# ai-dynamo/dynamo

Measured on AMD Instinct MI355X. Metric: output tok/s (node), Llama-3-70B serving, ISL8192/OSL1024, conc 16/GPU, higher is better.
Workload: dtype bf16; 1 GPU; model=llama-3-70b, global_batch=16, seq_len=8192, osl=1024, parallelism=agg1, kv_cache_dtype=auto

## Files before the change

### dynamo_amd/csrc/bindings.cpp

```cpp
#include <torch/extension.h>
#include <pybind11/pybind11.h>

namespace py = pybind11;

void rmsnorm(torch::Tensor out, torch::Tensor input, torch::Tensor weight, double eps);
void fused_add_rmsnorm(torch::Tensor input, torch::Tensor residual,
                       torch::Tensor weight, double eps);
void rope_append_qkv(torch::Tensor q_out, torch::Tensor kcache,
                     torch::Tensor vcache, torch::Tensor qkv,
                     c10::optional<torch::Tensor> bias,
                     torch::Tensor positions, torch::Tensor slot_mapping,
                     torch::Tensor cos_sin_cache, bool v_transposed);
void rope_inplace(torch::Tensor q, torch::Tensor k, torch::Tensor positions,
                  torch::Tensor cos_sin_cache, int64_t num_q_heads,
                  int64_t num_k_heads, int64_t head_dim);
void silu_mul(torch::Tensor out, torch::Tensor gate_up);
void gelu(torch::Tensor out, torch::Tensor input);
void kv_cache_append(torch::Tensor kcache, torch::Tensor vcache, torch::Tensor k,
                     torch::Tensor v, torch::Tensor slot_mapping,
                     bool v_transposed);
void gather_pages(torch::Tensor staging, torch::Tensor cache, torch::Tensor page_ids);
void scatter_pages(torch::Tensor staging, torch::Tensor cache, torch::Tensor page_ids);
void copy_pages(torch::Tensor dst_cache, torch::Tensor src_cache, torch::Tensor pairs);
int64_t paged_decode_num_chunks(int64_t max_ctx);
int64_t decode_chunk_tokens_py(int64_t max_ctx);
void paged_attention_decode(torch::Tensor out, torch::Tensor q, torch::Tensor kcache,
                            torch::Tensor vcache, torch::Tensor page_table,
                            torch::Tensor ctx_lens, torch::Tensor partial,
                            torch::Tensor ml, double scale,
                            int64_t chunk_tokens, bool v_transposed,
                            c10::optional<torch::Tensor> chunk_cnt);
void attention_prefill_paged(torch::Tensor out, torch::Tensor q,
                             torch::Tensor kcache, torch::Tensor vcache,
                             torch::Tensor page_table, torch::Tensor tile_seq,
                             torch::Tensor tile_q0, torch::Tensor seq_q_start,
                             torch::Tensor seq_q_len, torch::Tensor seq_ctx_len,
                             double scale, bool v_transposed);
void greedy_sample(torch::Tensor out, torch::Tensor logits);
void topkp_sample(torch::Tensor out, torch::Tensor logits,
                  torch::Tensor inv_temp, torch::Tensor top_k,
                  torch::Tensor top_p, int64_t seed,
                  c10::optional<torch::Tensor> row_seeds);
void gumbel_sample(torch::Tensor out, torch::Tensor logits, torch::Tensor inv_temp,
                   int64_t seed, c10::optional<torch::Tensor> row_seeds);
void moe_grouped_gemm(torch::Tensor y, torch::Tensor x, torch::Tensor w,
                      torch::Tensor tiles);
void moe_grouped_gemm_seg(torch::Tensor y, torch::Tensor x, torch::Tensor w,
                          torch::Tensor seg_start, int64_t max_tokens);
void topk_gating(torch::Tensor topw, torch::Tensor topi, torch::Tensor logits);
torch::Tensor ipc_alloc(int64_t nbytes, int64_t device);
py::bytes ipc_export(torch::Tensor t);
torch::Tensor ipc_open(py::bytes handle_bytes, int64_t nbytes, int64_t device);
void enable_peer_access(int64_t device, int64_t peer);
torch::Tensor mfma_probe(torch::Tensor A, torch::Tensor B);
torch::Tensor tr16_probe();
torch::Tensor vstage_probe();
torch::Tensor pv_probe(int64_t hot);

PYBIND11_MODULE(TORCH_EXTENSION_NAME, m) {
  m.doc() = "dynamo_amd native MI355X (gfx950) kernels";
  m.def("rmsnorm", &rmsnorm);
  m.def("fused_add_rmsnorm", &fused_add_rmsnorm);
  m.def("rope_inplace", &rope_inplace);
  m.def("rope_append_qkv", &rope_append_qkv,
        py::arg("q_out"), py::arg("kcache"), py::arg("vcache"),
        py::arg("qkv"), py::arg("bias"), py::arg("positions"),
        py::arg("slot_mapping"), py::arg("cos_sin"),
        py::arg("v_transposed") = false);
  m.def("silu_mul", &silu_mul);
  m.def("gelu", &gelu);
  m.def("kv_cache_append", &kv_cache_append, py::arg("kcache"),
        py::arg("vcache"), py::arg("k"), py::arg("v"),
        py::arg("slot_mapping"), py::arg("v_transposed") = false);
  m.def("gather_pages", &gather_pages);
  m.def("scatter_pages", &scatter_pages);
  m.def("copy_pages", &copy_pages);
  m.def("paged_decode_num_chunks", &paged_decode_num_chunks);
  m.def("decode_chunk_tokens", &decode_chunk_tokens_py);
  m.def("paged_attention_decode", &paged_attention_decode,
        py::arg("out"), py::arg("q"), py::arg("kcache"), py::arg("vcache"),
        py::arg("page_table"), py::arg("ctx_lens"), py::arg("partial"),
        py::arg("ml"), py::arg("scale"), py::arg("chunk_tokens"),
        py::arg("v_transposed") = false,
        py::arg("chunk_cnt") = py::none());
  m.def("attention_prefill_paged", &attention_prefill_paged,
        py::arg("out"), py::arg("q"), py::arg("kcache"), py::arg("vcache"),
        py::arg("page_table"), py::arg("tile_seq"), py::arg("tile_q0"),
        py::arg("seq_q_start"), py::arg("seq_q_len"), py::arg("seq_ctx_len"),
        py::arg("scale"), py::arg("v_transposed") = false);
  m.def("greedy_sample", &greedy_sample);
  m.def("gumbel_sample", &gumbel_sample, py::arg("out"), py::arg("logits"),
        py::arg("inv_temp"), py::arg("seed"),
        py::arg("row_seeds") = py::none());
  m.def("topkp_sample", &topkp_sample, py::arg("out"), py::arg("logits"),
        py::arg("inv_temp"), py::arg("top_k"), py::arg("top_p"),
        py::arg("seed"), py::arg("row_seeds") = py::none());
  m.def("moe_grouped_gemm", &moe_grouped_gemm);
  m.def("moe_grouped_gemm_seg", &moe_grouped_gemm_seg);
  m.def("topk_gating", &topk_gating);
  m.def("ipc_alloc", &ipc_alloc);
  m.def("ipc_export", &ipc_export);
  m.def("ipc_open", &ipc_open);
  m.def("enable_peer_access", &enable_peer_access);
  m.def("mfma_probe", &mfma_probe);
  m.def("tr16_probe", &tr16_probe);
  m.def("vstage_probe", &vstage_probe);
  m.def("pv_probe", &pv_probe);
}
```

### dynamo_amd/csrc/norm.hip

```cpp
#include "common.h"
#include <torch/extension.h>
#include <ATen/hip/HIPContext.h>

namespace {

constexpr int kBlock = 256;

template <bool FUSED_ADD>
__global__ void rmsnorm_kernel(short* __restrict__ out,
                               short* __restrict__ x,
                               short* __restrict__ res,
                               const short* __restrict__ w,
                               float eps, int rows, int D) {
  __shared__ float lds[kBlock / WAVE_SIZE];
  const int nvec = D / 8;
  for (int row = blockIdx.x; row < rows; row += gridDim.x) {
    short* xrow = x + (int64_t)row * D;
    short* rrow = FUSED_ADD ? res + (int64_t)row * D : nullptr;
    short* orow = out + (int64_t)row * D;

    float ss = 0.f;
    for (int v = threadIdx.x; v < nvec; v += kBlock) {
      short8 xv = *reinterpret_cast<const short8*>(xrow + v * 8);
      if constexpr (FUSED_ADD) {
        short8 rv = *reinterpret_cast<const short8*>(rrow + v * 8);
        short8 sv;
#pragma unroll
        for (int i = 0; i < 8; i++) {
          float s = bf16_to_f32(xv[i]) + bf16_to_f32(rv[i]);
          sv[i] = f32_to_bf16(s);
          ss += s * s;
        }
        *reinterpret_cast<short8*>(rrow + v * 8) = sv;
      } else {
#pragma unroll
        for (int i = 0; i < 8; i++) {
          float xf = bf16_to_f32(xv[i]);
          ss += xf * xf;
        }
      }
    }
    ss = block_reduce_sum(ss, lds);
    const float inv = rsqrtf(ss / (float)D + eps);

    for (int v = threadIdx.x; v < nvec; v += kBlock) {
      const short* src = FUSED_ADD ? rrow : xrow;
      short8 sv = *reinterpret_cast<const short8*>(src + v * 8);
      short8 wv = *reinterpret_cast<const short8*>(w + v * 8);
      short8 ov;
#pragma unroll
      for (int i = 0; i < 8; i++)
        ov[i] = f32_to_bf16(bf16_to_f32(sv[i]) * inv * bf16_to_f32(wv[i]));
      *reinterpret_cast<short8*>(orow + v * 8) = ov;
    }
    __syncthreads();
  }
}

}

void rmsnorm(torch::Tensor out, torch::Tensor input, torch::Tensor weight, double eps) {
  TORCH_CHECK(input.is_cuda() && input.dtype() == torch::kBFloat16);
  TORCH_CHECK(input.is_contiguous() && out.is_contiguous());
  const int D = input.size(-1);
  const int rows = input.numel() / D;
  TORCH_CHECK(D % 8 == 0, "hidden size must be a multiple of 8");
  const int grid = std::min<int>(rows, 2048);
  if (rows == 0) return;
  auto stream = at::cuda::getCurrentHIPStream();
  rmsnorm_kernel<false><<<grid, kBlock, 0, stream>>>(
      (short*)out.data_ptr(), (short*)input.data_ptr(), nullptr,
      (const short*)weight.data_ptr(), (float)eps, rows, D);
  HIP_CHECK_KERNEL();
}

void fused_add_rmsnorm(torch::Tensor input, torch::Tensor residual,
                       torch::Tensor weight, double eps) {
  TORCH_CHECK(input.is_cuda() && input.dtype() == torch::kBFloat16);
  TORCH_CHECK(input.is_contiguous() && residual.is_contiguous());
  const int D = input.size(-1);
  const int rows = input.numel() / D;
  TORCH_CHECK(D % 8 == 0);
  const int grid = std::min<int>(rows, 2048);
  if (rows == 0) return;
  auto stream = at::cuda::getCurrentHIPStream();
  rmsnorm_kernel<true><<<grid, kBlock, 0, stream>>>(
      (short*)input.data_ptr(), (short*)input.data_ptr(),
      (short*)residual.data_ptr(), (const short*)weight.data_ptr(),
      (float)eps, rows, D);
  HIP_CHECK_KERNEL();
}
```

### dynamo_amd/csrc/rope.hip

```cpp
#include "common.h"
#include <hip/hip_fp8.h>
#include <torch/extension.h>
#include <ATen/hip/HIPContext.h>

namespace {

constexpr int kBlock = 256;

__global__ void rope_kernel(short* __restrict__ q,
                            short* __restrict__ k,
                            const int32_t* __restrict__ positions,
                            const float* __restrict__ cos_sin,
                            int T, int Hq, int Hk, int hd) {
  const int t = blockIdx.x;
  if (t >= T) return;
  const int half = hd / 2;
  const int pos = positions[t];
  const float* cs = cos_sin + (int64_t)pos * hd;

  const int total = (Hq + Hk) * (half / 8);
  for (int idx = threadIdx.x; idx < total; idx += kBlock) {
    const int h = idx / (half / 8);
    const int i0 = (idx % (half / 8)) * 8;
    short* base = (h < Hq) ? q + ((int64_t)t * Hq + h) * hd
                           : k + ((int64_t)t * Hk + (h - Hq)) * hd;
    short8 x1 = *reinterpret_cast<const short8*>(base + i0);
    short8 x2 = *reinterpret_cast<const short8*>(base + half + i0);
    float4v c0 = *reinterpret_cast<const float4v*>(cs + i0);
    float4v c1 = *reinterpret_cast<const float4v*>(cs + i0 + 4);
    float4v s0 = *reinterpret_cast<const float4v*>(cs + half + i0);
    float4v s1 = *reinterpret_cast<const float4v*>(cs + half + i0 + 4);
    short8 o1, o2;
#pragma unroll
    for (int i = 0; i < 8; i++) {
      float c = (i < 4) ? c0[i] : c1[i - 4];
      float s = (i < 4) ? s0[i] : s1[i - 4];
      float a = bf16_to_f32(x1[i]);
      float b = bf16_to_f32(x2[i]);
      o1[i] = f32_to_bf16(a * c - b * s);
      o2[i] = f32_to_bf16(b * c + a * s);
    }
    *reinterpret_cast<short8*>(base + i0) = o1;
    *reinterpret_cast<short8*>(base + half + i0) = o2;
  }
}

template <int FP8 = 0, int VT = 0>
__global__ void rope_append_kernel(
    short* __restrict__ q_out,
    short* __restrict__ kcache,
    short* __restrict__ vcache,
    const short* __restrict__ qkv,
    const short* __restrict__ bias,
    const int32_t* __restrict__ positions,
    const int64_t* __restrict__ slots,
    const float* __restrict__ cos_sin,
    int T, int Hq, int Hkv, int page_size, int hd, int row_stride) {
  const int t = blockIdx.x;
  if (t >= T) return;
  const int half = hd / 2;
  const int pos = positions[t];
  const float* cs = cos_sin + (int64_t)pos * hd;
  const short* row = qkv + (int64_t)t * row_stride;
  const int64_t slot = slots[t];
  const int64_t page = slot >= 0 ? slot / page_size : 0;
  const int off = slot >= 0 ? (int)(slot % page_size) : 0;

  const int rope_units = (Hq + Hkv) * (half / 8);
  for (int idx = threadIdx.x; idx < rope_units; idx += kBlock) {
    const int h = idx / (half / 8);
    const int i0 = (idx % (half / 8)) * 8;
    const int src_off = h * hd;
    short8 x1 = *reinterpret_cast<const short8*>(row + src_off + i0);
    short8 x2 = *reinterpret_cast<const short8*>(row + src_off + half + i0);
    float4v c0 = *reinterpret_cast<const float4v*>(cs + i0);
    float4v c1 = *reinterpret_cast<const float4v*>(cs + i0 + 4);
    float4v s0 = *reinterpret_cast<const float4v*>(cs + half + i0);
    float4v s1 = *reinterpret_cast<const float4v*>(cs + half + i0 + 4);
    short8 o1, o2;
#pragma unroll
    for (int i = 0; i < 8; i++) {
      const float c = (i < 4) ? c0[i] : c1[i - 4];
      const float s = (i < 4) ? s0[i] : s1[i - 4];
      float a = bf16_to_f32(x1[i]);
      float b = bf16_to_f32(x2[i]);
      if (bias) {
        a += bf16_to_f32(bias[src_off + i0 + i]);
        b += bf16_to_f32(bias[src_off + half + i0 + i]);
      }
      o1[i] = f32_to_bf16(a * c - b * s);
      o2[i] = f32_to_bf16(b * c + a * s);
    }
    if (h < Hq) {
      short* qb = q_out + ((int64_t)t * Hq + h) * hd;
      *reinterpret_cast<short8*>(qb + i0) = o1;
      *reinterpret_cast<short8*>(qb + half + i0) = o2;
    } else if (slot >= 0) {
      const int kh = h - Hq;
      const int64_t kb = ((page * Hkv + kh) * page_size + off) * hd;
      if constexpr (FP8) {
        unsigned char* kc8 = reinterpret_cast<unsigned char*>(kcache);
        uchar8 p1, p2;
#pragma unroll
        for (int e = 0; e < 8; e++) {
          p1[e] = __hip_cvt_float_to_fp8(bf16_to_f32(o1[e]),
                                         __HIP_SATFINITE, __HIP_E4M3);
          p2[e] = __hip_cvt_float_to_fp8(bf16_to_f32(o2[e]),
                                         __HIP_SATFINITE, __HIP_E4M3);
        }
        *reinterpret_cast<uchar8*>(kc8 + kb + i0) = p1;
        *reinterpret_cast<uchar8*>(kc8 + kb + half + i0) = p2;
      } else {
        *reinterpret_cast<short8*>(kcache + kb + i0) = o1;
        *reinterpret_cast<short8*>(kcache + kb + half + i0) = o2;
      }
    }
  }
  if (slot >= 0) {
    const int voff = (Hq + Hkv) * hd;
    const int nvec = Hkv * hd / 8;
    for (int i = threadIdx.x; i < nvec; i += kBlock) {
      const int h = (i * 8) / hd;
      const int d = (i * 8) % hd;
      short8 v = *reinterpret_cast<const short8*>(row + voff + h * hd + d);
      if (bias) {
#pragma unroll
        for (int e = 0; e < 8; e++)
          v[e] = f32_to_bf16(bf16_to_f32(v[e]) +
                             bf16_to_f32(bias[voff + h * hd + d + e]));
      }
      if constexpr (VT) {
        const int64_t vb0 = ((page * Hkv + h) * hd + d) * page_size + off;
#pragma unroll
        for (int e = 0; e < 8; e++) {
          if constexpr (FP8) {
            reinterpret_cast<unsigned char*>(vcache)[vb0 + (int64_t)e *
                                                     page_size] =
                __hip_cvt_float_to_fp8(bf16_to_f32(v[e]), __HIP_SATFINITE,
                                       __HIP_E4M3);
          } else {
            vcache[vb0 + (int64_t)e * page_size] = v[e];
          }
        }
        continue;
      }
      const int64_t vb = ((page * Hkv + h) * page_size + off) * hd + d;
      if constexpr (FP8) {
        uchar8 pv;
#pragma unroll
        for (int e = 0; e < 8; e++)
          pv[e] = __hip_cvt_float_to_fp8(bf16_to_f32(v[e]),
                                         __HIP_SATFINITE, __HIP_E4M3);
        *reinterpret_cast<uchar8*>(
            reinterpret_cast<unsigned char*>(vcache) + vb) = pv;
      } else {
        *reinterpret_cast<short8*>(vcache + vb) = v;
      }
    }
  }
}

}

void rope_append_qkv(torch::Tensor q_out, torch::Tensor kcache,
                     torch::Tensor vcache, torch::Tensor qkv,
                     c10::optional<torch::Tensor> bias,
                     torch::Tensor positions, torch::Tensor slot_mapping,
                     torch::Tensor cos_sin_cache, bool v_transposed) {
  TORCH_CHECK(qkv.is_cuda() && qkv.dtype() == torch::kBFloat16);
  TORCH_CHECK(qkv.dim() == 2 && qkv.stride(1) == 1);
  TORCH_CHECK(positions.dtype() == torch::kInt32);
  TORCH_CHECK(slot_mapping.dtype() == torch::kInt64);
  TORCH_CHECK(cos_sin_cache.dtype() == torch::kFloat32);
  const int T = qkv.size(0);
  const int Hkv = kcache.size(1);
  const int page_size = kcache.size(2);
  const int hd = kcache.size(3);
  const int Hq = q_out.numel() / (T ? (int64_t)T * hd : hd);
  TORCH_CHECK(hd % 16 == 0 && (hd / 2) % 8 == 0);
  TORCH_CHECK(qkv.size(1) >= (Hq + 2 * Hkv) * hd);
  const short* bp = nullptr;
  if (bias.has_value()) {
    TORCH_CHECK(bias->numel() == (Hq + 2 * Hkv) * hd &&
                bias->dtype() == torch::kBFloat16 && bias->is_contiguous());
    bp = (const short*)bias->data_ptr();
  }
  if (T == 0) return;
  const bool fp8 = kcache.dtype() == torch::kFloat8_e4m3fn;
  TORCH_CHECK(fp8 || kcache.dtype() == torch::kBFloat16,
              "kv cache must be bf16 or float8_e4m3fn");
  auto stream = at::cuda::getCurrentHIPStream();
  auto launch = [&](auto kern) {
    kern<<<T, kBlock, 0, stream>>>(
        (short*)q_out.data_ptr(), (short*)kcache.data_ptr(),
        (short*)vcache.data_ptr(), (const short*)qkv.data_ptr(), bp,
        positions.data_ptr<int32_t>(), slot_mapping.data_ptr<int64_t>(),
        cos_sin_cache.data_ptr<float>(), T, Hq, Hkv, page_size, hd,
        (int)qkv.stride(0));
  };
  if (v_transposed)
    TORCH_CHECK(vcache.size(2) == hd && vcache.size(3) == page_size,
                "v_transposed expects vcache [P, Hkv, hd, ps]");
  if (fp8 && v_transposed) launch(rope_append_kernel<1, 1>);
  else if (fp8) launch(rope_append_kernel<1, 0>);
  else if (v_transposed) launch(rope_append_kernel<0, 1>);
  else launch(rope_append_kernel<0, 0>);
  HIP_CHECK_KERNEL();
}

void rope_inplace(torch::Tensor q, torch::Tensor k, torch::Tensor positions,
                  torch::Tensor cos_sin_cache, int64_t num_q_heads,
                  int64_t num_k_heads, int64_t head_dim) {
  TORCH_CHECK(q.is_cuda() && q.dtype() == torch::kBFloat16);
  TORCH_CHECK(positions.dtype() == torch::kInt32);
  TORCH_CHECK(cos_sin_cache.dtype() == torch::kFloat32);
  TORCH_CHECK(head_dim % 16 == 0, "head_dim must be a multiple of 16");
  const int T = q.numel() / (num_q_heads * head_dim);
  if (T == 0) return;
  auto stream = at::cuda::getCurrentHIPStream();
  rope_kernel<<<T, kBlock, 0, stream>>>(
      (short*)q.data_ptr(), (short*)k.data_ptr(),
      positions.data_ptr<int32_t>(), cos_sin_cache.data_ptr<float>(),
      T, (int)num_q_heads, (int)num_k_heads, (int)head_dim);
  HIP_CHECK_KERNEL();
}
```

### dynamo_amd/csrc/sampling.hip

```cpp
#include "common.h"
#include <torch/extension.h>
#include <ATen/hip/HIPContext.h>

namespace {

constexpr int kBlock = 512;

DEVINL uint64_t hash_u64(uint64_t x) {
  x += 0x9e3779b97f4a7c15ull;
  x = (x ^ (x >> 30)) * 0xbf58476d1ce4e5b9ull;
  x = (x ^ (x >> 27)) * 0x94d049bb133111ebull;
  return x ^ (x >> 31);
}

template <bool GUMBEL>
__global__ void sample_kernel(int32_t* __restrict__ out,
                              const float* __restrict__ logits,
                              const float* __restrict__ inv_temp,
                              uint64_t seed,
                              const uint64_t* __restrict__ row_seeds,
                              int V) {
  const int b = blockIdx.x;
  const float* row = logits + (int64_t)b * V;
  const float it = GUMBEL ? inv_temp[b] : 1.f;
  const uint64_t rs = row_seeds ? row_seeds[b] : (seed ^ ((uint64_t)b << 32));

  float best = -1e38f;
  int besti = -1;
  for (int v = threadIdx.x; v < V; v += kBlock) {
    float x = row[v] * it;
    if constexpr (GUMBEL) {
      const uint64_t h = hash_u64(rs ^ (uint64_t)v);
      const float u = (float)((h >> 11) + 1) * 4.8828125e-4f * 2.2737367544323206e-13f;
      x += -__logf(-__logf(u));
    }
    if (x > best || (x == best && v < besti)) { best = x; besti = v; }
  }
#pragma unroll
  for (int off = 32; off > 0; off >>= 1) {
    const float ob = __shfl_xor(best, off, WAVE_SIZE);
    const int oi = __shfl_xor(besti, off, WAVE_SIZE);
    if (ob > best || (ob == best && oi < besti)) { best = ob; besti = oi; }
  }
  __shared__ float sb[kBlock / WAVE_SIZE];
  __shared__ int si[kBlock / WAVE_SIZE];
  const int wid = threadIdx.x / WAVE_SIZE;
  if ((threadIdx.x & 63) == 0) { sb[wid] = best; si[wid] = besti; }
  __syncthreads();
  if (threadIdx.x == 0) {
    for (int w = 1; w < kBlock / WAVE_SIZE; w++) {
      if (sb[w] > best || (sb[w] == best && si[w] < besti)) { best = sb[w]; besti = si[w]; }
    }
    out[b] = besti;
  }
}

__global__ __launch_bounds__(kBlock) void topkp_sample_kernel(
    int32_t* __restrict__ out,
    const float* __restrict__ logits,
    const float* __restrict__ inv_temp,
    const int32_t* __restrict__ top_k,
    const float* __restrict__ top_p,
    uint64_t seed,
    const uint64_t* __restrict__ row_seeds,
    int V) {
  const int b = blockIdx.x;
  const uint64_t rs = row_seeds ? row_seeds[b] : (seed ^ ((uint64_t)b << 32));
  const float* row = logits + (int64_t)b * V;
  const int k = top_k[b];
  const float p = top_p[b];
  const bool use_k = (k > 0 && k < V);
  const bool use_p = (p < 1.0f);
  constexpr int kWaves = kBlock / WAVE_SIZE;
  __shared__ float red[kWaves];
  __shared__ float red2[kWaves];
  __shared__ float bcast[2];

  float m = -1e38f;
  for (int v = threadIdx.x; v < V; v += kBlock) m = fmaxf(m, row[v]);
  m = wave_reduce_max(m);
  if ((threadIdx.x & 63) == 0) red[threadIdx.x / WAVE_SIZE] = m;
  __syncthreads();
  if (threadIdx.x == 0) {
    for (int w = 1; w < kWaves; w++) m = fmaxf(m, red[w]);
    bcast[0] = m;
  }
  __syncthreads();
  m = bcast[0];

  float z = 0.f;
  for (int v = threadIdx.x; v < V; v += kBlock) z += __expf(row[v] - m);
  z = wave_reduce_sum(z);
  if ((threadIdx.x & 63) == 0) red[threadIdx.x / WAVE_SIZE] = z;
  __syncthreads();
  if (threadIdx.x == 0) {
    for (int w = 1; w < kWaves; w++) z += red[w];
    bcast[0] = z;
  }
  __syncthreads();
  const float inv_z = 1.f / bcast[0];

  float lo_k = 0.f, hi_k = 1.f, lo_p = 0.f, hi_p = 1.f;
  if (use_k || use_p) {
    for (int it = 0; it < 24; it++) {
      const float mid_k = 0.5f * (lo_k + hi_k);
      const float mid_p = 0.5f * (lo_p + hi_p);
      float cnt = 0.f, mass = 0.f;
      for (int v = threadIdx.x; v < V; v += kBlock) {
        const float pv = __expf(row[v] - m) * inv_z;
        if (use_k && pv >= mid_k) cnt += 1.f;
        if (use_p && pv >= mid_p) mass += pv;
      }
      cnt = wave_reduce_sum(cnt);
      mass = wave_reduce_sum(mass);
      const int wid = threadIdx.x / WAVE_SIZE;
      if ((threadIdx.x & 63) == 0) { red[wid] = cnt; red2[wid] = mass; }
      __syncthreads();
      if (threadIdx.x == 0) {
        for (int w = 1; w < kWaves; w++) { cnt += red[w]; mass += red2[w]; }
        bcast[0] = cnt;
        bcast[1] = mass;
      }
      __syncthreads();
      cnt = bcast[0];
      mass = bcast[1];
      if (use_k) { if (cnt >= (float)k) lo_k = mid_k; else hi_k = mid_k; }
      if (use_p) { if (mass >= p) lo_p = mid_p; else hi_p = mid_p; }
      __syncthreads();
    }
  }
  const float thr = fmaxf(use_k ? lo_k : 0.f, use_p ? lo_p : 0.f);

  const float it_ = inv_temp[b];
  float best = -1e38f;
  int besti = -1;
  for (int v = threadIdx.x; v < V; v += kBlock) {
    const float pv = __expf(row[v] - m) * inv_z;
    if (pv < thr) continue;
    const uint64_t h = hash_u64(rs ^ (uint64_t)v);
    const float u = (float)((h >> 11) + 1) * 4.8828125e-4f * 2.2737367544323206e-13f;
    const float x = row[v] * it_ + -__logf(-__logf(u));
    if (x > best || (x == best && v < besti)) { best = x; besti = v; }
  }
#pragma unroll
  for (int off = 32; off > 0; off >>= 1) {
    const float ob = __shfl_xor(best, off, WAVE_SIZE);
    const int oi = __shfl_xor(besti, off, WAVE_SIZE);
    if (ob > best || (ob == best && oi != -1 && (besti == -1 || oi < besti))) {
      best = ob; besti = oi;
    }
  }
  __shared__ float sb2[kWaves];
  __shared__ int si2[kWaves];
  const int wid = threadIdx.x / WAVE_SIZE;
  if ((threadIdx.x & 63) == 0) { sb2[wid] = best; si2[wid] = besti; }
  __syncthreads();
  if (threadIdx.x == 0) {
    for (int w = 1; w < kWaves; w++) {
      if (sb2[w] > best || (sb2[w] == best && si2[w] != -1 &&
                            (besti == -1 || si2[w] < besti))) {
        best = sb2[w]; besti = si2[w];
      }
    }
    out[b] = besti;
  }
}

}

void greedy_sample(torch::Tensor out, torch::Tensor logits) {
  TORCH_CHECK(logits.is_cuda() && logits.dtype() == torch::kFloat32);
  TORCH_CHECK(out.dtype() == torch::kInt32);
  const int B = logits.size(0);
  const int V = logits.size(1);
  if (B == 0) return;
  auto stream = at::cuda::getCurrentHIPStream();
  sample_kernel<false><<<B, kBlock, 0, stream>>>(
      out.data_ptr<int32_t>(), logits.data_ptr<float>(), nullptr, 0, nullptr,
      V);
  HIP_CHECK_KERNEL();
}

static const uint64_t* opt_seeds(const c10::optional<torch::Tensor>& t,
                                 int B) {
  if (!t.has_value()) return nullptr;
  TORCH_CHECK(t->dtype() == torch::kInt64 && t->numel() == B &&
              t->is_cuda() && t->is_contiguous());
  return reinterpret_cast<const uint64_t*>(t->data_ptr<int64_t>());
}

void gumbel_sample(torch::Tensor out, torch::Tensor logits, torch::Tensor inv_temp,
                   int64_t seed, c10::optional<torch::Tensor> row_seeds) {
  TORCH_CHECK(logits.is_cuda() && logits.dtype() == torch::kFloat32);
  TORCH_CHECK(inv_temp.dtype() == torch::kFloat32);
  const int B = logits.size(0);
  const int V = logits.size(1);
  if (B == 0) return;
  auto stream = at::cuda::getCurrentHIPStream();
  sample_kernel<true><<<B, kBlock, 0, stream>>>(
      out.data_ptr<int32_t>(), logits.data_ptr<float>(),
      inv_temp.data_ptr<float>(), (uint64_t)seed, opt_seeds(row_seeds, B), V);
  HIP_CHECK_KERNEL();
}

void topkp_sample(torch::Tensor out, torch::Tensor logits,
                  torch::Tensor inv_temp, torch::Tensor top_k,
                  torch::Tensor top_p, int64_t seed,
                  c10::optional<torch::Tensor> row_seeds) {
  TORCH_CHECK(logits.is_cuda() && logits.dtype() == torch::kFloat32);
  TORCH_CHECK(inv_temp.dtype() == torch::kFloat32);
  TORCH_CHECK(top_k.dtype() == torch::kInt32);
  TORCH_CHECK(top_p.dtype() == torch::kFloat32);
  const int B = logits.size(0);
  const int V = logits.size(1);
  TORCH_CHECK(top_k.numel() == B && top_p.numel() == B && inv_temp.numel() == B);
  if (B == 0) return;
  auto stream = at::cuda::getCurrentHIPStream();
  topkp_sample_kernel<<<B, kBlock, 0, stream>>>(
      out.data_ptr<int32_t>(), logits.data_ptr<float>(),
      inv_temp.data_ptr<float>(), top_k.data_ptr<int32_t>(),
      top_p.data_ptr<float>(), (uint64_t)seed, opt_seeds(row_seeds, B), V);
  HIP_CHECK_KERNEL();
}
```

### dynamo_amd/ops/__init__.py

```python
from __future__ import annotations

import torch

from . import torch_ref
from .torch_ref import make_cos_sin_cache

_hip_mod = None
_hip_err: Exception | None = None


def hip():
    global _hip_mod, _hip_err
    if _hip_mod is None:
        try:
            from dynamo_amd import _hip as m
            _hip_mod = m
        except Exception as e:
            _hip_err = e
            raise RuntimeError(
                "dynamo_amd._hip native extension is not available on a GPU "
                "device path. Build it with `python setup.py build_ext "
                f"--inplace` (PYTORCH_ROCM_ARCH=gfx950). Original error: {e}"
            ) from e
    return _hip_mod


def hip_available() -> bool:
    try:
        hip()
        return True
    except RuntimeError:
        return False


def rmsnorm(x: torch.Tensor, weight: torch.Tensor, eps: float) -> torch.Tensor:
    if x.is_cuda:
        out = torch.empty_like(x)
        hip().rmsnorm(out, x.contiguous(), weight, eps)
        return out
    return torch_ref.rmsnorm(x, weight, eps)


def fused_add_rmsnorm(x, residual, weight, eps):
    if x.is_cuda:
        hip().fused_add_rmsnorm(x, residual, weight, eps)
        return x
    return torch_ref.fused_add_rmsnorm(x, residual, weight, eps)


def rope_inplace(q, k, positions, cos_sin, num_q_heads, num_k_heads, head_dim):
    if q.is_cuda:
        hip().rope_inplace(q, k, positions, cos_sin, num_q_heads, num_k_heads,
                           head_dim)
        return q, k
    return torch_ref.rope(q, k, positions, cos_sin, num_q_heads, num_k_heads,
                          head_dim)


def silu_mul(gate_up: torch.Tensor) -> torch.Tensor:
    if gate_up.is_cuda:
        d = gate_up.shape[-1] // 2
        out = torch.empty(gate_up.shape[:-1] + (d,), dtype=gate_up.dtype,
                          device=gate_up.device)
        hip().silu_mul(out, gate_up.contiguous())
        return out
    return torch_ref.silu_mul(gate_up)


def gelu(x: torch.Tensor) -> torch.Tensor:
    if x.is_cuda:
        out = torch.empty_like(x)
        hip().gelu(out, x.contiguous())
        return out
    return torch_ref.gelu(x)


def kv_cache_append(kcache, vcache, k, v, slot_mapping,
                    v_transposed=False):
    if kcache.is_cuda:
        hip().kv_cache_append(kcache, vcache, k.contiguous(), v.contiguous(),
                              slot_mapping, v_transposed)
    else:
        torch_ref.kv_cache_append(kcache, vcache, k, v, slot_mapping,
                                  v_transposed)


def rope_append_qkv(qkv, bias, positions, slot_mapping, cos_sin,
                    kcache, vcache, num_q_heads, num_kv_heads, head_dim,
                    v_transposed=False):
    T = qkv.shape[0]
    if qkv.is_cuda:
        q_out = torch.empty(T, num_q_heads * head_dim, dtype=qkv.dtype,
                            device=qkv.device)
        hip().rope_append_qkv(q_out, kcache, vcache, qkv, bias, positions,
                              slot_mapping, cos_sin, v_transposed)
        return q_out
    if bias is not None:
        qkv = qkv + bias
    q, k, v = qkv.split([num_q_heads * head_dim, num_kv_heads * head_dim,
                         num_kv_heads * head_dim], dim=-1)
    q = q.contiguous()
    k = k.contiguous()
    q, k = torch_ref.rope(q, k, positions, cos_sin, num_q_heads,
                          num_kv_heads, head_dim)
    torch_ref.kv_cache_append(kcache, vcache, k.view(T, num_kv_heads, head_dim),
                              v.view(T, num_kv_heads, head_dim), slot_mapping,
                              v_transposed)
    return q


class DecodeScratch:

    def __init__(self, max_batch: int, num_q_heads: int, head_dim: int,
                 max_ctx: int, device):
        self.chunks = int(hip().paged_decode_num_chunks(max_ctx))
        self.chunk_tokens = int(hip().decode_chunk_tokens(max_ctx))
        self.partial = torch.empty(max_batch, num_q_heads, self.chunks, head_dim,
                                   dtype=torch.float32, device=device)
        self.ml = torch.empty(max_batch, num_q_heads, self.chunks, 2,
                              dtype=torch.float32, device=device)
        self.chunk_cnt = torch.zeros(max_batch * 128, dtype=torch.int32,
                                     device=device)

    def view(self, batch: int):
        return self.partial[:batch], self.ml[:batch]


def paged_attention_decode(q, kcache, vcache, page_table, ctx_lens, scale,
                           scratch: "DecodeScratch | None" = None, out=None,
                           v_transposed=False):
    if q.is_cuda:
        if out is None:
            out = torch.empty_like(q)
        assert scratch is not None, "GPU decode needs a DecodeScratch"
        partial, ml = scratch.view(q.shape[0])
        hip().paged_attention_decode(out, q, kcache, vcache, page_table,
                                     ctx_lens, partial, ml, scale,
                                     scratch.chunk_tokens, v_transposed,
                                     scratch.chunk_cnt)
        return out
    r = torch_ref.paged_attention_decode(q, kcache, vcache, page_table,
                                         ctx_lens, scale,
                                         v_transposed=v_transposed)
    if out is not None:
        out.copy_(r)
        return out
    return r


def prefill_tile_rows(num_q_heads: int, num_kv_heads: int) -> int:
    if num_q_heads % num_kv_heads == 0:
        g = num_q_heads // num_kv_heads
        if g in (2, 4, 8):
            return (8 // g) * 32
    return 64


def build_prefill_tiles(seq_q_lens, device, rows: int = 64):
    tile_seq, tile_q0 = [], []
    for s, ql in enumerate(seq_q_lens):
        for q0 in range(0, int(ql), rows):
            tile_seq.append(s)
            tile_q0.append(q0)
    return (torch.tensor(tile_seq, dtype=torch.int32, device=device),
            torch.tensor(tile_q0, dtype=torch.int32, device=device))


def attention_prefill_paged(q, kcache, vcache, page_table, seq_q_start,
                            seq_q_len, seq_ctx_len, scale, tiles=None,
                            v_transposed=False):
    if q.is_cuda:
        out = torch.empty_like(q)
        if tiles is None:
            rows = prefill_tile_rows(q.shape[1], kcache.shape[1])
            tiles = build_prefill_tiles(seq_q_len.tolist(), q.device, rows)
        tile_seq, tile_q0 = tiles
        hip().attention_prefill_paged(out, q, kcache, vcache, page_table,
                                      tile_seq, tile_q0, seq_q_start,
                                      seq_q_len, seq_ctx_len, scale,
                                      v_transposed)
        return out
    return torch_ref.attention_prefill_paged(q, kcache, vcache, page_table,
                                             seq_q_start, seq_q_len,
                                             seq_ctx_len, scale,
                                             v_transposed=v_transposed)


def greedy_sample(logits: torch.Tensor) -> torch.Tensor:
    if logits.is_cuda:
        out = torch.empty(logits.shape[0], dtype=torch.int32,
                          device=logits.device)
        hip().greedy_sample(out, logits.float().contiguous())
        return out
    return torch_ref.greedy_sample(logits)


def _splitmix64(x: torch.Tensor) -> torch.Tensor:
    def lsr(v, k):
        return (v >> k) & ((1 << (64 - k)) - 1)
    x = x + 0x9e3779b97f4a7c15
    x = (x ^ lsr(x, 30)) * -0x40a7b892e31b1a47
    x = (x ^ lsr(x, 27)) * -0x6b2fb644ecceee15
    return x ^ lsr(x, 31)


def gumbel_sample(logits: torch.Tensor, inv_temp: torch.Tensor,
                  seed: int, row_seeds: torch.Tensor = None) -> torch.Tensor:
    if logits.is_cuda:
        out = torch.empty(logits.shape[0], dtype=torch.int32,
                          device=logits.device)
        hip().gumbel_sample(out, logits.float().contiguous(), inv_temp, seed,
                            row_seeds)
        return out
    B, V = logits.shape
    if row_seeds is None:
        rs = (torch.tensor(seed, dtype=torch.int64)
              ^ (torch.arange(B, dtype=torch.int64) << 32))
    else:
        rs = row_seeds.to(torch.int64).cpu()
    v = torch.arange(V, dtype=torch.int64).unsqueeze(0)
    h = _splitmix64(rs.unsqueeze(1) ^ v)
    u = (((h >> 11) & ((1 << 53) - 1)) + 1).double() * (2.0 ** -53)
    g = -torch.log(-torch.log(u.float()))
    return (logits.float() * inv_temp.unsqueeze(-1) + g).argmax(-1).to(torch.int32)


def topkp_sample(logits: torch.Tensor, inv_temp: torch.Tensor,
                 top_k: torch.Tensor, top_p: torch.Tensor,
                 seed: int, row_seeds: torch.Tensor = None) -> torch.Tensor:
    out = torch.empty(logits.shape[0], dtype=torch.int32,
                      device=logits.device)
    hip().topkp_sample(out, logits.float().contiguous(), inv_temp,
                       top_k, top_p, seed, row_seeds)
    return out


def topk_gating(logits: torch.Tensor, k: int):
    if logits.is_cuda:
        T = logits.shape[0]
        topw = torch.empty(T, k, dtype=torch.float32, device=logits.device)
        topi = torch.empty(T, k, dtype=torch.int32, device=logits.device)
        hip().topk_gating(topw, topi, logits.float().contiguous())
        return topw, topi
    p = torch.softmax(logits.float(), dim=-1)
    topw, topi = torch.topk(p, k, dim=-1)
    return topw / topw.sum(-1, keepdim=True), topi.to(torch.int32)


def build_moe_tiles(counts, max_m: int = 16):
    tiles = []
    r0 = 0
    for e, n in enumerate(counts):
        off = 0
        while off < n:
            m = min(max_m, n - off)
            tiles.append((e, r0 + off, m))
            off += m
        r0 += n
    return tiles


def moe_grouped_gemm(x: torch.Tensor, w: torch.Tensor, tiles_t: torch.Tensor):
    y = torch.empty(x.shape[0], w.shape[1], dtype=x.dtype, device=x.device)
    hip().moe_grouped_gemm(y, x.contiguous(), w, tiles_t)
    return y


def moe_grouped_gemm_seg(x, w, seg_start, max_tokens):
    y = torch.empty(x.shape[0], w.shape[1], dtype=x.dtype, device=x.device)
    hip().moe_grouped_gemm_seg(y, x.contiguous(), w, seg_start, max_tokens)
    return y


def gather_pages(staging, cache, page_ids):
    if cache.is_cuda:
        hip().gather_pages(staging, cache, page_ids)
    else:
        n = page_ids.shape[0]
        pe = cache[0].numel()
        staging.view(-1)[: n * pe] = cache[page_ids.long()].reshape(-1)


def scatter_pages(staging, cache, page_ids):
    if cache.is_cuda:
        hip().scatter_pages(staging, cache, page_ids)
    else:
        n = page_ids.shape[0]
        pe = cache[0].numel()
        cache[page_ids.long()] = staging.view(-1)[: n * pe].view(n, *cache.shape[1:])


def copy_pages(dst_cache, src_cache, pairs):
    if src_cache.is_cuda:
        hip().copy_pages(dst_cache, src_cache, pairs)
    else:
        src = pairs[:, 0].long()
        dst = pairs[:, 1].long()
        dst_cache[dst] = src_cache[src]
```

Before: 424.0 tok/s.

## Add fast-path kernels for rmsnorm, rope-append and sampling

Adds a register-resident rmsnorm variant that caches weights in registers and unrolls per-thread vectors when the hidden size divides evenly. It also adds a rope/KV-append kernel that spreads each token across several blocks for small token counts, and a vectorized, unrolled float4 scan for greedy and Gumbel sampling. All three are enabled by default through new allow_fast flags. They target launch and latency-bound small decode kernels, at the cost of extra template instantiations and separate code paths to keep correct.

```diff
diff --git a/dynamo_amd/csrc/bindings.cpp b/dynamo_amd/csrc/bindings.cpp
--- a/dynamo_amd/csrc/bindings.cpp
+++ b/dynamo_amd/csrc/bindings.cpp
@@ -3,14 +3,16 @@
 
 namespace py = pybind11;
 
-void rmsnorm(torch::Tensor out, torch::Tensor input, torch::Tensor weight, double eps);
+void rmsnorm(torch::Tensor out, torch::Tensor input, torch::Tensor weight,
+             double eps, bool allow_fast);
 void fused_add_rmsnorm(torch::Tensor input, torch::Tensor residual,
-                       torch::Tensor weight, double eps);
+                       torch::Tensor weight, double eps, bool allow_fast);
 void rope_append_qkv(torch::Tensor q_out, torch::Tensor kcache,
                      torch::Tensor vcache, torch::Tensor qkv,
                      c10::optional<torch::Tensor> bias,
                      torch::Tensor positions, torch::Tensor slot_mapping,
-                     torch::Tensor cos_sin_cache, bool v_transposed);
+                     torch::Tensor cos_sin_cache, bool v_transposed,
+                     bool allow_fast);
 void rope_inplace(torch::Tensor q, torch::Tensor k, torch::Tensor positions,
                   torch::Tensor cos_sin_cache, int64_t num_q_heads,
                   int64_t num_k_heads, int64_t head_dim);
@@ -36,13 +38,14 @@
                              torch::Tensor tile_q0, torch::Tensor seq_q_start,
                              torch::Tensor seq_q_len, torch::Tensor seq_ctx_len,
                              double scale, bool v_transposed);
-void greedy_sample(torch::Tensor out, torch::Tensor logits);
+void greedy_sample(torch::Tensor out, torch::Tensor logits, bool allow_fast);
 void topkp_sample(torch::Tensor out, torch::Tensor logits,
                   torch::Tensor inv_temp, torch::Tensor top_k,
                   torch::Tensor top_p, int64_t seed,
                   c10::optional<torch::Tensor> row_seeds);
 void gumbel_sample(torch::Tensor out, torch::Tensor logits, torch::Tensor inv_temp,
-                   int64_t seed, c10::optional<torch::Tensor> row_seeds);
+                   int64_t seed, c10::optional<torch::Tensor> row_seeds,
+                   bool allow_fast);
 void moe_grouped_gemm(torch::Tensor y, torch::Tensor x, torch::Tensor w,
                       torch::Tensor tiles);
 void moe_grouped_gemm_seg(torch::Tensor y, torch::Tensor x, torch::Tensor w,
@@ -59,14 +62,17 @@
 
 PYBIND11_MODULE(TORCH_EXTENSION_NAME, m) {
   m.doc() = "dynamo_amd native MI355X (gfx950) kernels";
-  m.def("rmsnorm", &rmsnorm);
-  m.def("fused_add_rmsnorm", &fused_add_rmsnorm);
+  m.def("rmsnorm", &rmsnorm, py::arg("out"), py::arg("input"),
+        py::arg("weight"), py::arg("eps"), py::arg("allow_fast") = true);
+  m.def("fused_add_rmsnorm", &fused_add_rmsnorm, py::arg("input"),
+        py::arg("residual"), py::arg("weight"), py::arg("eps"),
+        py::arg("allow_fast") = true);
   m.def("rope_inplace", &rope_inplace);
   m.def("rope_append_qkv", &rope_append_qkv,
         py::arg("q_out"), py::arg("kcache"), py::arg("vcache"),
         py::arg("qkv"), py::arg("bias"), py::arg("positions"),
         py::arg("slot_mapping"), py::arg("cos_sin"),
-        py::arg("v_transposed") = false);
+        py::arg("v_transposed") = false, py::arg("allow_fast") = true);
   m.def("silu_mul", &silu_mul);
   m.def("gelu", &gelu);
   m.def("kv_cache_append", &kv_cache_append, py::arg("kcache"),
@@ -88,10 +94,11 @@
         py::arg("page_table"), py::arg("tile_seq"), py::arg("tile_q0"),
         py::arg("seq_q_start"), py::arg("seq_q_len"), py::arg("seq_ctx_len"),
         py::arg("scale"), py::arg("v_transposed") = false);
-  m.def("greedy_sample", &greedy_sample);
+  m.def("greedy_sample", &greedy_sample, py::arg("out"), py::arg("logits"),
+        py::arg("allow_fast") = true);
   m.def("gumbel_sample", &gumbel_sample, py::arg("out"), py::arg("logits"),
         py::arg("inv_temp"), py::arg("seed"),
-        py::arg("row_seeds") = py::none());
+        py::arg("row_seeds") = py::none(), py::arg("allow_fast") = true);
   m.def("topkp_sample", &topkp_sample, py::arg("out"), py::arg("logits"),
         py::arg("inv_temp"), py::arg("top_k"), py::arg("top_p"),
         py::arg("seed"), py::arg("row_seeds") = py::none());
diff --git a/dynamo_amd/csrc/norm.hip b/dynamo_amd/csrc/norm.hip
--- a/dynamo_amd/csrc/norm.hip
+++ b/dynamo_amd/csrc/norm.hip
@@ -57,36 +57,121 @@
   }
 }
 
+template <bool FUSED_ADD, int VPT>
+__global__ __launch_bounds__(kBlock) void rmsnorm_reg_kernel(
+    short* __restrict__ out,
+    short* __restrict__ x,
+    short* __restrict__ res,
+    const short* __restrict__ w,
+    float eps, int rows) {
+  __shared__ float lds[kBlock / WAVE_SIZE];
+  constexpr int D = 8 * kBlock * VPT;
+  short8 wv[VPT];
+#pragma unroll
+  for (int j = 0; j < VPT; j++)
+    wv[j] = *reinterpret_cast<const short8*>(w + (threadIdx.x + j * kBlock) * 8);
+  for (int row = blockIdx.x; row < rows; row += gridDim.x) {
+    short* xrow = x + (int64_t)row * D;
+    short* rrow = FUSED_ADD ? res + (int64_t)row * D : nullptr;
+    short* orow = out + (int64_t)row * D;
+
+    short8 sv[VPT], rv[VPT];
+#pragma unroll
+    for (int j = 0; j < VPT; j++) {
+      const int v = threadIdx.x + j * kBlock;
+      sv[j] = *reinterpret_cast<const short8*>(xrow + v * 8);
+      if constexpr (FUSED_ADD)
+        rv[j] = *reinterpret_cast<const short8*>(rrow + v * 8);
+    }
+    float ss = 0.f;
+#pragma unroll
+    for (int j = 0; j < VPT; j++) {
+      if constexpr (FUSED_ADD) {
+#pragma unroll
+        for (int i = 0; i < 8; i++) {
+          float s = bf16_to_f32(sv[j][i]) + bf16_to_f32(rv[j][i]);
+          sv[j][i] = f32_to_bf16(s);
+          ss += s * s;
+        }
+        *reinterpret_cast<short8*>(rrow + (threadIdx.x + j * kBlock) * 8) = sv[j];
+      } else {
+#pragma unroll
+        for (int i = 0; i < 8; i++) {
+          float xf = bf16_to_f32(sv[j][i]);
+          ss += xf * xf;
+        }
+      }
+    }
+    ss = block_reduce_sum(ss, lds);
+    const float inv = rsqrtf(ss / (float)D + eps);
+
+#pragma unroll
+    for (int j = 0; j < VPT; j++) {
+      short8 ov;
+#pragma unroll
+      for (int i = 0; i < 8; i++)
+        ov[i] = f32_to_bf16(bf16_to_f32(sv[j][i]) * inv * bf16_to_f32(wv[j][i]));
+      *reinterpret_cast<short8*>(orow + (threadIdx.x + j * kBlock) * 8) = ov;
+    }
+    __syncthreads();
+  }
 }
 
-void rmsnorm(torch::Tensor out, torch::Tensor input, torch::Tensor weight, double eps) {
+template <bool FUSED_ADD>
+void launch_rmsnorm(short* out, short* x, short* res, const short* w,
+                    float eps, int rows, int D, bool allow_fast,
+                    hipStream_t stream) {
+  const int grid = std::min<int>(rows, 2048);
+  const int nvec = D / 8;
+  const int vpt = (allow_fast && nvec % kBlock == 0) ? nvec / kBlock : 0;
+  switch (vpt) {
+    case 1:
+      rmsnorm_reg_kernel<FUSED_ADD, 1><<<grid, kBlock, 0, stream>>>(
+          out, x, res, w, eps, rows);
+      break;
+    case 2:
+      rmsnorm_reg_kernel<FUSED_ADD, 2><<<grid, kBlock, 0, stream>>>(
+          out, x, res, w, eps, rows);
+      break;
+    case 4:
+      rmsnorm_reg_kernel<FUSED_ADD, 4><<<grid, kBlock, 0, stream>>>(
+          out, x, res, w, eps, rows);
+      break;
+    default:
+      rmsnorm_kernel<FUSED_ADD><<<grid, kBlock, 0, stream>>>(
+          out, x, res, w, eps, rows, D);
+  }
+}
+
+}
+
+void rmsnorm(torch::Tensor out, torch::Tensor input, torch::Tensor weight,
+             double eps, bool allow_fast) {
   TORCH_CHECK(input.is_cuda() && input.dtype() == torch::kBFloat16);
   TORCH_CHECK(input.is_contiguous() && out.is_contiguous());
   const int D = input.size(-1);
   const int rows = input.numel() / D;
   TORCH_CHECK(D % 8 == 0, "hidden size must be a multiple of 8");
-  const int grid = std::min<int>(rows, 2048);
   if (rows == 0) return;
   auto stream = at::cuda::getCurrentHIPStream();
-  rmsnorm_kernel<false><<<grid, kBlock, 0, stream>>>(
-      (short*)out.data_ptr(), (short*)input.data_ptr(), nullptr,
-      (const short*)weight.data_ptr(), (float)eps, rows, D);
+  launch_rmsnorm<false>((short*)out.data_ptr(), (short*)input.data_ptr(),
+                        nullptr, (const short*)weight.data_ptr(), (float)eps,
+                        rows, D, allow_fast, stream);
   HIP_CHECK_KERNEL();
 }
 
 void fused_add_rmsnorm(torch::Tensor input, torch::Tensor residual,
-                       torch::Tensor weight, double eps) {
+                       torch::Tensor weight, double eps, bool allow_fast) {
   TORCH_CHECK(input.is_cuda() && input.dtype() == torch::kBFloat16);
   TORCH_CHECK(input.is_contiguous() && residual.is_contiguous());
   const int D = input.size(-1);
   const int rows = input.numel() / D;
   TORCH_CHECK(D % 8 == 0);
-  const int grid = std::min<int>(rows, 2048);
   if (rows == 0) return;
   auto stream = at::cuda::getCurrentHIPStream();
-  rmsnorm_kernel<true><<<grid, kBlock, 0, stream>>>(
-      (short*)input.data_ptr(), (short*)input.data_ptr(),
-      (short*)residual.data_ptr(), (const short*)weight.data_ptr(),
-      (float)eps, rows, D);
+  launch_rmsnorm<true>((short*)input.data_ptr(), (short*)input.data_ptr(),
+                       (short*)residual.data_ptr(),
+                       (const short*)weight.data_ptr(), (float)eps, rows, D,
+                       allow_fast, stream);
   HIP_CHECK_KERNEL();
 }
diff --git a/dynamo_amd/csrc/rope.hip b/dynamo_amd/csrc/rope.hip
--- a/dynamo_amd/csrc/rope.hip
+++ b/dynamo_amd/csrc/rope.hip
@@ -6,6 +6,7 @@
 namespace {
 
 constexpr int kBlock = 256;
+constexpr int kUnitMaxTokens = 256;
 
 __global__ void rope_kernel(short* __restrict__ q,
                             short* __restrict__ k,
@@ -160,13 +161,138 @@
   }
 }
 
+template <int FP8 = 0, int VT = 0>
+__global__ __launch_bounds__(kBlock) void rope_append_unit_kernel(
+    short* __restrict__ q_out,
+    short* __restrict__ kcache,
+    short* __restrict__ vcache,
+    const short* __restrict__ qkv,
+    const short* __restrict__ bias,
+    const int32_t* __restrict__ positions,
+    const int64_t* __restrict__ slots,
+    const float* __restrict__ cos_sin,
+    int T, int Hq, int Hkv, int page_size, int hd, int row_stride) {
+  const int t = blockIdx.x;
+  const int idx = blockIdx.y * kBlock + threadIdx.x;
+  const int half = hd / 2;
+  const short* row = qkv + (int64_t)t * row_stride;
+  const int rope_units = (Hq + Hkv) * (half / 8);
+
+  if (idx < rope_units) {
+    const int h = idx / (half / 8);
+    const int i0 = (idx % (half / 8)) * 8;
+    const int src_off = h * hd;
+    short8 x1 = *reinterpret_cast<const short8*>(row + src_off + i0);
+    short8 x2 = *reinterpret_cast<const short8*>(row + src_off + half + i0);
+    short8 b1 = {}, b2 = {};
+    if (bias) {
+      b1 = *reinterpret_cast<const short8*>(bias + src_off + i0);
+      b2 = *reinterpret_cast<const short8*>(bias + src_off + half + i0);
+    }
+    const int pos = positions[t];
+    const float* cs = cos_sin + (int64_t)pos * hd;
+    float4v c0 = *reinterpret_cast<const float4v*>(cs + i0);
+    float4v c1 = *reinterpret_cast<const float4v*>(cs + i0 + 4);
+    float4v s0 = *reinterpret_cast<const float4v*>(cs + half + i0);
+    float4v s1 = *reinterpret_cast<const float4v*>(cs + half + i0 + 4);
+    const int64_t slot = slots[t];
+    short8 o1, o2;
+#pragma unroll
+    for (int i = 0; i < 8; i++) {
+      const float c = (i < 4) ? c0[i] : c1[i - 4];
+      const float s = (i < 4) ? s0[i] : s1[i - 4];
+      float a = bf16_to_f32(x1[i]);
+      float b = bf16_to_f32(x2[i]);
+      if (bias) {
+        a += bf16_to_f32(b1[i]);
+        b += bf16_to_f32(b2[i]);
+      }
+      o1[i] = f32_to_bf16(a * c - b * s);
+      o2[i] = f32_to_bf16(b * c + a * s);
+    }
+    if (h < Hq) {
+      short* qb = q_out + ((int64_t)t * Hq + h) * hd;
+      *reinterpret_cast<short8*>(qb + i0) = o1;
+      *reinterpret_cast<short8*>(qb + half + i0) = o2;
+    } else if (slot >= 0) {
+      const int64_t page = slot / page_size;
+      const int off = (int)(slot % page_size);
+      const int kh = h - Hq;
+      const int64_t kb = ((page * Hkv + kh) * page_size + off) * hd;
+      if constexpr (FP8) {
+        unsigned char* kc8 = reinterpret_cast<unsigned char*>(kcache);
+        uchar8 p1, p2;
+#pragma unroll
+        for (int e = 0; e < 8; e++) {
+          p1[e] = __hip_cvt_float_to_fp8(bf16_to_f32(o1[e]),
+                                         __HIP_SATFINITE, __HIP_E4M3);
+          p2[e] = __hip_cvt_float_to_fp8(bf16_to_f32(o2[e]),
+                                         __HIP_SATFINITE, __HIP_E4M3);
+        }
+        *reinterpret_cast<uchar8*>(kc8 + kb + i0) = p1;
+        *reinterpret_cast<uchar8*>(kc8 + kb + half + i0) = p2;
+      } else {
+        *reinterpret_cast<short8*>(kcache + kb + i0) = o1;
+        *reinterpret_cast<short8*>(kcache + kb + half + i0) = o2;
+      }
+    }
+    return;
+  }
+
+  const int i = idx - rope_units;
+  if (i >= Hkv * hd / 8) return;
+  const int voff = (Hq + Hkv) * hd;
+  const int h = (i * 8) / hd;
+  const int d = (i * 8) % hd;
+  short8 v = *reinterpret_cast<const short8*>(row + voff + h * hd + d);
+  short8 bv = {};
+  if (bias) bv = *reinterpret_cast<const short8*>(bias + voff + h * hd + d);
+  const int64_t slot = slots[t];
+  if (slot < 0) return;
+  const int64_t page = slot / page_size;
+  const int off = (int)(slot % page_size);
+  if (bias) {
+#pragma unroll
+    for (int e = 0; e < 8; e++)
+      v[e] = f32_to_bf16(bf16_to_f32(v[e]) + bf16_to_f32(bv[e]));
+  }
+  if constexpr (VT) {
+    const int64_t vb0 = ((page * Hkv + h) * hd + d) * page_size + off;
+#pragma unroll
+    for (int e = 0; e < 8; e++) {
+      if constexpr (FP8) {
+        reinterpret_cast<unsigned char*>(vcache)[vb0 + (int64_t)e *
+                                                 page_size] =
+            __hip_cvt_float_to_fp8(bf16_to_f32(v[e]), __HIP_SATFINITE,
+                                   __HIP_E4M3);
+      } else {
+        vcache[vb0 + (int64_t)e * page_size] = v[e];
+      }
+    }
+    return;
+  }
+  const int64_t vb = ((page * Hkv + h) * page_size + off) * hd + d;
+  if constexpr (FP8) {
+    uchar8 pv;
+#pragma unroll
+    for (int e = 0; e < 8; e++)
+      pv[e] = __hip_cvt_float_to_fp8(bf16_to_f32(v[e]),
+                                     __HIP_SATFINITE, __HIP_E4M3);
+    *reinterpret_cast<uchar8*>(
+        reinterpret_cast<unsigned char*>(vcache) + vb) = pv;
+  } else {
+    *reinterpret_cast<short8*>(vcache + vb) = v;
+  }
+}
+
 }
 
 void rope_append_qkv(torch::Tensor q_out, torch::Tensor kcache,
                      torch::Tensor vcache, torch::Tensor qkv,
                      c10::optional<torch::Tensor> bias,
                      torch::Tensor positions, torch::Tensor slot_mapping,
-                     torch::Tensor cos_sin_cache, bool v_transposed) {
+                     torch::Tensor cos_sin_cache, bool v_transposed,
+                     bool allow_fast) {
   TORCH_CHECK(qkv.is_cuda() && qkv.dtype() == torch::kBFloat16);
   TORCH_CHECK(qkv.dim() == 2 && qkv.stride(1) == 1);
   TORCH_CHECK(positions.dtype() == torch::kInt32);
@@ -190,8 +316,12 @@
   TORCH_CHECK(fp8 || kcache.dtype() == torch::kBFloat16,
               "kv cache must be bf16 or float8_e4m3fn");
   auto stream = at::cuda::getCurrentHIPStream();
+  const int units = (Hq + Hkv) * (hd / 16) + Hkv * hd / 8;
+  const bool unit = allow_fast && T <= kUnitMaxTokens &&
+                    reinterpret_cast<uintptr_t>(bp) % 16 == 0;
+  const dim3 grid = unit ? dim3(T, (units + kBlock - 1) / kBlock) : dim3(T);
   auto launch = [&](auto kern) {
-    kern<<<T, kBlock, 0, stream>>>(
+    kern<<<grid, kBlock, 0, stream>>>(
         (short*)q_out.data_ptr(), (short*)kcache.data_ptr(),
         (short*)vcache.data_ptr(), (const short*)qkv.data_ptr(), bp,
         positions.data_ptr<int32_t>(), slot_mapping.data_ptr<int64_t>(),
@@ -201,10 +331,17 @@
   if (v_transposed)
     TORCH_CHECK(vcache.size(2) == hd && vcache.size(3) == page_size,
                 "v_transposed expects vcache [P, Hkv, hd, ps]");
-  if (fp8 && v_transposed) launch(rope_append_kernel<1, 1>);
-  else if (fp8) launch(rope_append_kernel<1, 0>);
-  else if (v_transposed) launch(rope_append_kernel<0, 1>);
-  else launch(rope_append_kernel<0, 0>);
+  if (unit) {
+    if (fp8 && v_transposed) launch(rope_append_unit_kernel<1, 1>);
+    else if (fp8) launch(rope_append_unit_kernel<1, 0>);
+    else if (v_transposed) launch(rope_append_unit_kernel<0, 1>);
+    else launch(rope_append_unit_kernel<0, 0>);
+  } else {
+    if (fp8 && v_transposed) launch(rope_append_kernel<1, 1>);
+    else if (fp8) launch(rope_append_kernel<1, 0>);
+    else if (v_transposed) launch(rope_append_kernel<0, 1>);
+    else launch(rope_append_kernel<0, 0>);
+  }
   HIP_CHECK_KERNEL();
 }
 
diff --git a/dynamo_amd/csrc/sampling.hip b/dynamo_amd/csrc/sampling.hip
--- a/dynamo_amd/csrc/sampling.hip
+++ b/dynamo_amd/csrc/sampling.hip
@@ -5,6 +5,7 @@
 namespace {
 
 constexpr int kBlock = 512;
+constexpr int kScanUnroll = 8;
 
 DEVINL uint64_t hash_u64(uint64_t x) {
   x += 0x9e3779b97f4a7c15ull;
@@ -14,12 +15,25 @@
 }
 
 template <bool GUMBEL>
-__global__ void sample_kernel(int32_t* __restrict__ out,
-                              const float* __restrict__ logits,
-                              const float* __restrict__ inv_temp,
-                              uint64_t seed,
-                              const uint64_t* __restrict__ row_seeds,
-                              int V) {
+DEVINL void sample_consider(float logit, int v, float it, uint64_t rs,
+                            float& best, int& besti) {
+  float x = logit * it;
+  if constexpr (GUMBEL) {
+    const uint64_t h = hash_u64(rs ^ (uint64_t)v);
+    const float u = (float)((h >> 11) + 1) * 4.8828125e-4f * 2.2737367544323206e-13f;
+    x += -__logf(-__logf(u));
+  }
+  if (x > best || (x == best && v < besti)) { best = x; besti = v; }
+}
+
+template <bool GUMBEL, bool FAST>
+__global__ __launch_bounds__(kBlock) void sample_kernel(
+    int32_t* __restrict__ out,
+    const float* __restrict__ logits,
+    const float* __restrict__ inv_temp,
+    uint64_t seed,
+    const uint64_t* __restrict__ row_seeds,
+    int V) {
   const int b = blockIdx.x;
   const float* row = logits + (int64_t)b * V;
   const float it = GUMBEL ? inv_temp[b] : 1.f;
@@ -27,14 +41,37 @@
 
   float best = -1e38f;
   int besti = -1;
-  for (int v = threadIdx.x; v < V; v += kBlock) {
-    float x = row[v] * it;
-    if constexpr (GUMBEL) {
-      const uint64_t h = hash_u64(rs ^ (uint64_t)v);
-      const float u = (float)((h >> 11) + 1) * 4.8828125e-4f * 2.2737367544323206e-13f;
-      x += -__logf(-__logf(u));
-    }
-    if (x > best || (x == best && v < besti)) { best = x; besti = v; }
+  if constexpr (FAST) {
+    const int mis = (int)((reinterpret_cast<uintptr_t>(row) >> 2) & 3);
+    const int head = min(V, (4 - mis) & 3);
+    const int n4 = (V - head) / 4;
+    const float4v* row4 = reinterpret_cast<const float4v*>(row + head);
+    for (int i0 = 0; i0 < n4; i0 += kScanUnroll * kBlock) {
+      float4v r[kScanUnroll];
+#pragma unroll
+      for (int u = 0; u < kScanUnroll; u++) {
+        const int i = i0 + u * kBlock + threadIdx.x;
+        if (i < n4) r[u] = row4[i];
+      }
+#pragma unroll
+      for (int u = 0; u < kScanUnroll; u++) {
+        const int i = i0 + u * kBlock + threadIdx.x;
+        if (i < n4) {
+#pragma unroll
+          for (int e = 0; e < 4; e++)
+            sample_consider<GUMBEL>(r[u][e], head + i * 4 + e, it, rs, best,
+                                    besti);
+        }
+      }
+    }
+    if ((int)threadIdx.x < head)
+      sample_consider<GUMBEL>(row[threadIdx.x], threadIdx.x, it, rs, best,
+                              besti);
+    const int v = head + n4 * 4 + threadIdx.x;
+    if (v < V) sample_consider<GUMBEL>(row[v], v, it, rs, best, besti);
+  } else {
+    for (int v = threadIdx.x; v < V; v += kBlock)
+      sample_consider<GUMBEL>(row[v], v, it, rs, best, besti);
   }
 #pragma unroll
   for (int off = 32; off > 0; off >>= 1) {
@@ -168,16 +205,18 @@
 
 }
 
-void greedy_sample(torch::Tensor out, torch::Tensor logits) {
+void greedy_sample(torch::Tensor out, torch::Tensor logits, bool allow_fast) {
   TORCH_CHECK(logits.is_cuda() && logits.dtype() == torch::kFloat32);
   TORCH_CHECK(out.dtype() == torch::kInt32);
   const int B = logits.size(0);
   const int V = logits.size(1);
   if (B == 0) return;
   auto stream = at::cuda::getCurrentHIPStream();
-  sample_kernel<false><<<B, kBlock, 0, stream>>>(
-      out.data_ptr<int32_t>(), logits.data_ptr<float>(), nullptr, 0, nullptr,
-      V);
+  auto kern = allow_fast ? sample_kernel<false, true>
+                         : sample_kernel<false, false>;
+  kern<<<B, kBlock, 0, stream>>>(out.data_ptr<int32_t>(),
+                                 logits.data_ptr<float>(), nullptr, 0, nullptr,
+                                 V);
   HIP_CHECK_KERNEL();
 }
 
@@ -190,14 +229,17 @@
 }
 
 void gumbel_sample(torch::Tensor out, torch::Tensor logits, torch::Tensor inv_temp,
-                   int64_t seed, c10::optional<torch::Tensor> row_seeds) {
+                   int64_t seed, c10::optional<torch::Tensor> row_seeds,
+                   bool allow_fast) {
   TORCH_CHECK(logits.is_cuda() && logits.dtype() == torch::kFloat32);
   TORCH_CHECK(inv_temp.dtype() == torch::kFloat32);
   const int B = logits.size(0);
   const int V = logits.size(1);
   if (B == 0) return;
   auto stream = at::cuda::getCurrentHIPStream();
-  sample_kernel<true><<<B, kBlock, 0, stream>>>(
+  auto kern = allow_fast ? sample_kernel<true, true>
+                         : sample_kernel<true, false>;
+  kern<<<B, kBlock, 0, stream>>>(
       out.data_ptr<int32_t>(), logits.data_ptr<float>(),
       inv_temp.data_ptr<float>(), (uint64_t)seed, opt_seeds(row_seeds, B), V);
   HIP_CHECK_KERNEL();
diff --git a/dynamo_amd/ops/__init__.py b/dynamo_amd/ops/__init__.py
--- a/dynamo_amd/ops/__init__.py
+++ b/dynamo_amd/ops/__init__.py
@@ -33,17 +33,18 @@
         return False
 
 
-def rmsnorm(x: torch.Tensor, weight: torch.Tensor, eps: float) -> torch.Tensor:
+def rmsnorm(x: torch.Tensor, weight: torch.Tensor, eps: float,
+            allow_fast: bool = True) -> torch.Tensor:
     if x.is_cuda:
         out = torch.empty_like(x)
-        hip().rmsnorm(out, x.contiguous(), weight, eps)
+        hip().rmsnorm(out, x.contiguous(), weight, eps, allow_fast)
         return out
     return torch_ref.rmsnorm(x, weight, eps)
 
 
-def fused_add_rmsnorm(x, residual, weight, eps):
+def fused_add_rmsnorm(x, residual, weight, eps, allow_fast=True):
     if x.is_cuda:
-        hip().fused_add_rmsnorm(x, residual, weight, eps)
+        hip().fused_add_rmsnorm(x, residual, weight, eps, allow_fast)
         return x
     return torch_ref.fused_add_rmsnorm(x, residual, weight, eps)
 
@@ -87,13 +88,13 @@
 
 def rope_append_qkv(qkv, bias, positions, slot_mapping, cos_sin,
                     kcache, vcache, num_q_heads, num_kv_heads, head_dim,
-                    v_transposed=False):
+                    v_transposed=False, allow_fast=True):
     T = qkv.shape[0]
     if qkv.is_cuda:
         q_out = torch.empty(T, num_q_heads * head_dim, dtype=qkv.dtype,
                             device=qkv.device)
         hip().rope_append_qkv(q_out, kcache, vcache, qkv, bias, positions,
-                              slot_mapping, cos_sin, v_transposed)
+                              slot_mapping, cos_sin, v_transposed, allow_fast)
         return q_out
     if bias is not None:
         qkv = qkv + bias
@@ -186,11 +187,11 @@
                                              v_transposed=v_transposed)
 
 
-def greedy_sample(logits: torch.Tensor) -> torch.Tensor:
+def greedy_sample(logits: torch.Tensor, allow_fast: bool = True) -> torch.Tensor:
     if logits.is_cuda:
         out = torch.empty(logits.shape[0], dtype=torch.int32,
                           device=logits.device)
-        hip().greedy_sample(out, logits.float().contiguous())
+        hip().greedy_sample(out, logits.float().contiguous(), allow_fast)
         return out
     return torch_ref.greedy_sample(logits)
 
@@ -205,12 +206,13 @@
 
 
 def gumbel_sample(logits: torch.Tensor, inv_temp: torch.Tensor,
-                  seed: int, row_seeds: torch.Tensor = None) -> torch.Tensor:
+                  seed: int, row_seeds: torch.Tensor = None,
+                  allow_fast: bool = True) -> torch.Tensor:
     if logits.is_cuda:
         out = torch.empty(logits.shape[0], dtype=torch.int32,
                           device=logits.device)
         hip().gumbel_sample(out, logits.float().contiguous(), inv_temp, seed,
-                            row_seeds)
+                            row_seeds, allow_fast)
         return out
     B, V = logits.shape
     if row_seeds is None:
```

Measured after the change: 431.0 tok/s, median of 6. +1.7%, better.
